# W-Ted/F3D-Gaus

Measured on AMD Instinct MI355X. Metric: rendered views/sec at 256x256 (N Gaussians, K cams), higher is better.
Workload: dtype f32; 1 GPU; C2: 1 image/GPU, 196608 Gaussians (sigma0=0.01), 120-view orbit @256x256, GOF forward raster only; timed region = render + 8-bit RGB frames copied to pinned host memory; compositing arithmetic: fast = error-free float32 pairs for the float64 island + hardware exp/rcp/rsq; every channel within 1e-4 of the oracle (RGB <= 3e-7), EXCEPT that the distortion channel (values 1e-7..1e-5 from cancelling fl; gaussians=196608, views=120, resolution=256, tile_cull=1, views_per_call=120, render_mode=fast, channels=all, parallelism=single GPU

## Files before the change

f3d-gaus_amd/csrc/f3dg_binning.hip:

```cpp
#include "f3dg_common.h"
#include "f3dg_scan.h"

namespace {

typedef unsigned long long u64;
typedef unsigned int u32;

__global__ void __launch_bounds__(F3DG_BLOCK)
scan_reduce_kernel(const u32* __restrict__ in, u64 n, u32* __restrict__ block_sums)
{
    __shared__ u32 wsum[F3DG_BLOCK / 64];
    const u64 base = (u64)blockIdx.x * F3DG_SCAN_CHUNK;
    u32 s = 0;
#pragma unroll
    for (int i = 0; i < F3DG_SCAN_ITEMS; i++) {
        const u64 k = base + (u64)i * F3DG_BLOCK + threadIdx.x;
        if (k < n) s += in[k];
    }
#pragma unroll
    for (int off = 32; off > 0; off >>= 1) s += __shfl_down(s, off, 64);
    if ((threadIdx.x & 63) == 0) wsum[threadIdx.x >> 6] = s;
    __syncthreads();
    if (threadIdx.x == 0) block_sums[blockIdx.x] = wsum[0] + wsum[1] + wsum[2] + wsum[3];
}

__global__ void __launch_bounds__(1024)
scan_blocksums_kernel(u32* __restrict__ block_sums, u32 nblocks, F3dgHeader* __restrict__ hdr)
{
    __shared__ u64 wtot[16];
    const u64 total = scan_array_in_place<16, 1, u64>(block_sums, nblocks, 0u, wtot);
    if (hdr) set_status(hdr, total);
}

__global__ void __launch_bounds__(F3DG_BLOCK)
scan_apply_kernel(const u32* in, u32* out , u64 n, const u32* __restrict__ block_sums,
                  int exclusive)
{
    __shared__ u32 wtot[F3DG_BLOCK / 64];
    const u64 base = (u64)blockIdx.x * F3DG_SCAN_CHUNK + (u64)threadIdx.x * F3DG_SCAN_ITEMS;
    u32 v[F3DG_SCAN_ITEMS];
    u32 s = 0;
    if (base + F3DG_SCAN_ITEMS <= n) {
#pragma unroll
        for (int i = 0; i < F3DG_SCAN_ITEMS / 4; i++) {
            const uint4 w = reinterpret_cast<const uint4*>(in + base)[i];
            v[4 * i] = w.x; v[4 * i + 1] = w.y; v[4 * i + 2] = w.z; v[4 * i + 3] = w.w;
        }
    } else {
#pragma unroll
        for (int i = 0; i < F3DG_SCAN_ITEMS; i++) v[i] = (base + i < n) ? in[base + i] : 0;
    }
#pragma unroll
    for (int i = 0; i < F3DG_SCAN_ITEMS; i++) s += v[i];
    u32 run = block_sums[blockIdx.x] + block_scan_exclusive<F3DG_BLOCK / 64>(s, wtot);
    u32 o[F3DG_SCAN_ITEMS];
#pragma unroll
    for (int i = 0; i < F3DG_SCAN_ITEMS; i++) {
        const u32 before = run;
        run += v[i];
        o[i] = exclusive ? before : run;
    }
    if (base + F3DG_SCAN_ITEMS <= n) {
#pragma unroll
        for (int i = 0; i < F3DG_SCAN_ITEMS / 4; i++)
            reinterpret_cast<uint4*>(out + base)[i] = make_uint4(o[4 * i], o[4 * i + 1], o[4 * i + 2], o[4 * i + 3]);
    } else {
#pragma unroll
        for (int i = 0; i < F3DG_SCAN_ITEMS; i++)
            if (base + i < n) out[base + i] = o[i];
    }
}


struct SegChunk {
    u64 seg_base;
    u64 obase;
    u32 n;
    u32 cps;
    u32 c;
    u32 seg;
};

struct SegTable {
    const u32* vstart;
    const u32* bglob;
    const u32* xprefix;
    u32 xstride;
    u32 V;
};

struct ShiftDigit {
    int shift;
    u32 mask = 255u;
    __device__ __forceinline__ u32 operator()(u32 k) const { return (k >> shift) & mask; }
};
struct CompactDigit {
    u32 kbase;
    __device__ __forceinline__ u32 operator()(u32 k) const { const u32 d = (k - kbase) >> 16; return d < 255u ? d : 255u; }
};

template <typename K, typename DIGIT, bool MINMAX = false>
__device__ __forceinline__ void hist_chunk(const K* __restrict__ keys, const SegChunk& ck, const DIGIT digit, u32* __restrict__ hist,
                                           u32 (*h)[256], u32* __restrict__ minmax = nullptr)
{
    u32 kmin = 0xFFFFFFFFu, kmax = 0u;
#pragma unroll
    for (int w = 0; w < F3DG_BLOCK / 64; w++) h[w][threadIdx.x] = 0;
    __syncthreads();
    u32* hw = h[threadIdx.x >> 6];
    constexpr int VEC = 16 / (int)sizeof(K);
    typedef K __attribute__((ext_vector_type(VEC))) KV;
    const u64 base = (u64)ck.c * F3DG_SORT_CHUNK;
    const u64 g0 = ck.seg_base + base;
    const u64 g1 = ck.seg_base + ((u64)ck.n - base < (u64)F3DG_SORT_CHUNK ? (u64)ck.n : base + F3DG_SORT_CHUNK);
    for (u64 a = (g0 & ~(u64)(VEC - 1)) + (u64)threadIdx.x * VEC; a < g1; a += (u64)F3DG_BLOCK * VEC) {
        const KV w = *reinterpret_cast<const KV*>(keys + a);
#pragma unroll
        for (int q = 0; q < VEC; q++) {
            if (a + q >= g0 && a + q < g1) {
                const u32 key = (u32)w[q];
                atomicAdd(&hw[digit(key)], 1u);
                if (MINMAX && key != 0xFFFFFFFFu) { kmin = key < kmin ? key : kmin; kmax = key > kmax ? key : kmax; }
            }
        }
    }
    __shared__ u32 wmm[2][F3DG_BLOCK / 64];
    if (MINMAX) {
#pragma unroll
        for (int off = 32; off > 0; off >>= 1) {
            const u32 a = __shfl_down(kmin, off, 64), b = __shfl_down(kmax, off, 64);
            kmin = a < kmin ? a : kmin; kmax = b > kmax ? b : kmax;
        }
        if ((threadIdx.x & 63) == 0) { wmm[0][threadIdx.x >> 6] = kmin; wmm[1][threadIdx.x >> 6] = kmax; }
    }
    __syncthreads();
    if (MINMAX && threadIdx.x == 0) {
        u32 a = wmm[0][0], b = wmm[1][0];
#pragma unroll
        for (int w = 1; w < F3DG_BLOCK / 64; w++) { a = wmm[0][w] < a ? wmm[0][w] : a; b = wmm[1][w] > b ? wmm[1][w] : b; }
        minmax[0] = a; minmax[1] = b;
    }
    hist[ck.obase + (u64)threadIdx.x * ck.cps + ck.c] = h[0][threadIdx.x] + h[1][threadIdx.x] + h[2][threadIdx.x] + h[3][threadIdx.x];
}

struct ScatterShared {
    u32 cnt[F3DG_BLOCK / 64][256];
    u32 lbase[256];
    u32 gdelta[256];
    u32 wtot[F3DG_BLOCK / 64];
    u32 sval[F3DG_SORT_CHUNK];
};

template <typename K, bool IOTA, typename DIGIT>
__device__ __forceinline__ void scatter_chunk(const K* __restrict__ keys_in, const u32* __restrict__ vals_in, K* __restrict__ keys_out,
                                              u32* __restrict__ vals_out, const SegChunk& ck, const DIGIT digit,
                                              const u32* __restrict__ offsets , ScatterShared& sh, K* skey)
{
    const u32 n = ck.n;
    const u64 block_base = (u64)ck.c * F3DG_SORT_CHUNK;
    const u32 in_block = (u32)((n - block_base) < (u64)F3DG_SORT_CHUNK ? (n - block_base) : (u64)F3DG_SORT_CHUNK);
    const int lane = threadIdx.x & 63, wave = threadIdx.x >> 6;
#pragma unroll
    for (int w = 0; w < F3DG_BLOCK / 64; w++) sh.cnt[w][threadIdx.x] = 0;
    __syncthreads();

    const u64 wave_base = block_base + (u64)wave * (64 * F3DG_SORT_ITEMS);
    u32 key[F3DG_SORT_ITEMS];
    u32 val[F3DG_SORT_ITEMS];
    u32 rank[F3DG_SORT_ITEMS];
    const u64 lane_lt = ((u64)1 << lane) - 1;
#pragma unroll
    for (int r = 0; r < F3DG_SORT_ITEMS; r++) {
        const u64 i = wave_base + (u64)r * 64 + lane;
        const bool valid = i < n;
        key[r] = valid ? (u32)keys_in[ck.seg_base + i] : 0u;
        val[r] = IOTA ? (u32)i : (valid ? vals_in[ck.seg_base + i] : 0u);
    }
#pragma unroll
    for (int r = 0; r < F3DG_SORT_ITEMS; r++) {
        const u64 i = wave_base + (u64)r * 64 + lane;
        const bool valid = i < n;
        const u32 d = digit(key[r]);
        u64 diff = 0;
#pragma unroll
        for (int b = 0; b < 8; b++) {
            const u32 own = (u32)((int)(d << (31 - b)) >> 31);
            const u64 bal = __ballot(own != 0u);
            diff |= bal ^ (((u64)own << 32) | own);
        }
        const u64 same = __ballot(valid) & ~diff;
        const u32 below = (u32)__popcll(same & lane_lt);
        const u32 prev = sh.cnt[wave][d];
        rank[r] = prev + below;
        __builtin_amdgcn_wave_barrier();
        if (valid && below == 0) sh.cnt[wave][d] = prev + (u32)__popcll(same);
        __builtin_amdgcn_wave_barrier();
    }
    __syncthreads();
    {
        const u32 d = threadIdx.x;
        const u32 c0 = sh.cnt[0][d], c1 = sh.cnt[1][d], c2 = sh.cnt[2][d], c3 = sh.cnt[3][d];
        const u32 tot = c0 + c1 + c2 + c3;
        const u32 excl = block_scan_exclusive<F3DG_BLOCK / 64>(tot, sh.wtot);
        sh.lbase[d] = excl;
        sh.gdelta[d] = offsets[ck.obase + (u64)d * ck.cps + ck.c] - excl;
        sh.cnt[0][d] = excl;
        sh.cnt[1][d] = excl + c0;
        sh.cnt[2][d] = excl + c0 + c1;
        sh.cnt[3][d] = excl + c0 + c1 + c2;
    }
    __syncthreads();
#pragma unroll
    for (int r = 0; r < F3DG_SORT_ITEMS; r++) {
        const u64 i = wave_base + (u64)r * 64 + lane;
        if (i < n) {
            const u32 d = digit(key[r]);
            const u32 slot = sh.cnt[wave][d] + rank[r];
            skey[slot] = (K)key[r];
            sh.sval[slot] = val[r];
        }
    }
    __syncthreads();
    for (u32 slot = threadIdx.x; slot < in_block; slot += F3DG_BLOCK) {
        const K k = skey[slot];
        const u32 d = digit((u32)k);
        const u32 pos = sh.gdelta[d] + slot;
        if (keys_out) keys_out[pos] = k;
        vals_out[pos] = sh.sval[slot];
    }
}

__device__ __forceinline__ SegChunk fixed_chunk(u32 seg_len, u32 cps)
{
    u32 seg, c;
    f3dg_xcd_map(blockIdx.x, gridDim.x / cps, cps, seg, c);
    SegChunk ck;
    ck.seg_base = (u64)seg * seg_len; ck.obase = (u64)seg * 256u * cps; ck.n = seg_len; ck.cps = cps; ck.c = c; ck.seg = seg;
    return ck;
}

__device__ __forceinline__ bool gsort_compact(const u32* __restrict__ minmax, u32 view, u32& kbase)
{
    const u32 kmin = minmax[2 * view], kmax = minmax[2 * view + 1];
    kbase = kmin & 0xFFFF0000u;
    return kmin <= kmax && ((kmax - kbase) >> 24) == 0u;
}

template <int PASS>
__global__ void __launch_bounds__(F3DG_BLOCK)
gsort_hist_kernel(const u32* __restrict__ keys, u32 seg_len, u32 cps, u32* __restrict__ hist, const u32* __restrict__ minmax,
                  u32* __restrict__ chunk_minmax, int standin )
{
    __shared__ u32 h[F3DG_BLOCK / 64][256];
    const SegChunk ck = fixed_chunk(seg_len, cps);
    if constexpr (PASS == 0) {
        hist_chunk<u32, ShiftDigit>(keys, ck, ShiftDigit{0}, hist, h);
    } else if constexpr (PASS == 1) {
        hist_chunk<u32, ShiftDigit, true>(keys, ck, ShiftDigit{8}, hist, h, chunk_minmax + 2 * ((size_t)ck.seg * cps + ck.c));
    } else {
        u32 kbase;
        const bool compact = gsort_compact(minmax, ck.seg, kbase);
        if (!compact) {
            hist_chunk<u32, ShiftDigit>(keys, ck, ShiftDigit{8 * PASS}, hist, h);
        } else if constexpr (PASS == 2) {
            hist_chunk<u32, CompactDigit>(keys, ck, CompactDigit{kbase}, hist, h);
        } else if (standin) {
            const u64 base = (u64)ck.c * F3DG_SORT_CHUNK;
            const u32 in_chunk = (u32)((ck.n - base) < (u64)F3DG_SORT_CHUNK ? (ck.n - base) : (u64)F3DG_SORT_CHUNK);
            hist[ck.obase + (u64)threadIdx.x * ck.cps + ck.c] = threadIdx.x == 0 ? in_chunk : 0u;
        }
    }
}

__global__ void __launch_bounds__(1024)
gsort_scan_kernel(u32 n_per_seg , u32 seg_len, u32* __restrict__ hist, const u32* __restrict__ skip_compact )
{
    __shared__ u32 wtot[16];
    u32 kbase;
    if (skip_compact && gsort_compact(skip_compact, blockIdx.x, kbase)) return;
    scan_array_in_place<16, 4, u32>(hist + (size_t)blockIdx.x * n_per_seg, n_per_seg, blockIdx.x * seg_len, wtot);
}

__global__ void __launch_bounds__(64)
gsort_range_kernel(u32 cps, const u32* __restrict__ chunk_minmax, u32* __restrict__ minmax)
{
    u32 kmin = 0xFFFFFFFFu, kmax = 0u;
    for (u32 c = threadIdx.x; c < cps; c += 64) {
        const u32 a = chunk_minmax[2 * ((size_t)blockIdx.x * cps + c)], b = chunk_minmax[2 * ((size_t)blockIdx.x * cps + c) + 1];
        kmin = a < kmin ? a : kmin; kmax = b > kmax ? b : kmax;
    }
#pragma unroll
    for (int off = 32; off > 0; off >>= 1) {
        const u32 a = __shfl_down(kmin, off, 64), b = __shfl_down(kmax, off, 64);
        kmin = a < kmin ? a : kmin; kmax = b > kmax ? b : kmax;
    }
    if (threadIdx.x == 0) { minmax[2 * blockIdx.x] = kmin; minmax[2 * blockIdx.x + 1] = kmax; }
}

template <int PASS>
__global__ void __launch_bounds__(F3DG_BLOCK)
gsort_scatter_kernel(const u32* __restrict__ keys_in, const u32* __restrict__ vals_in, u32* __restrict__ keys_out,
                     u32* __restrict__ vals_out, u32 seg_len, u32 cps, const u32* __restrict__ offsets, const u32* __restrict__ minmax)
{
    __shared__ ScatterShared sh;
    __shared__ u32 skey[F3DG_SORT_CHUNK];
    const SegChunk ck = fixed_chunk(seg_len, cps);
    if constexpr (PASS == 0) {
        scatter_chunk<u32, true, ShiftDigit>(keys_in, vals_in, keys_out, vals_out, ck, ShiftDigit{0}, offsets, sh, skey);
    } else if constexpr (PASS == 1) {
        scatter_chunk<u32, false, ShiftDigit>(keys_in, vals_in, keys_out, vals_out, ck, ShiftDigit{8}, offsets, sh, skey);
    } else {
        u32 kbase;
        const bool compact = gsort_compact(minmax, ck.seg, kbase);
        if (!compact)
            scatter_chunk<u32, false, ShiftDigit>(keys_in, vals_in, PASS == 3 ? (u32*)nullptr : keys_out, vals_out, ck, ShiftDigit{8 * PASS}, offsets, sh, skey);
        else if constexpr (PASS == 2)
            scatter_chunk<u32, false, CompactDigit>(keys_in, vals_in, (u32*)nullptr, vals_out, ck, CompactDigit{kbase}, offsets, sh, skey);
    }
}


__global__ void __launch_bounds__(1024)
block_sums_scan_kernel(u32 nb, u32* __restrict__ block_sums, u64* __restrict__ view_total)
{
    __shared__ u64 wtot[16];
    const u64 total = scan_array_in_place<16, 1, u64>(block_sums + (size_t)blockIdx.x * nb, nb, 0u, wtot);
    if (threadIdx.x == 0) view_total[blockIdx.x] = total;
}

__global__ void __launch_bounds__(512)
view_segments_kernel(int V, const u64* __restrict__ view_total, F3dgHeader* __restrict__ hdr, u32* __restrict__ vstart,
                     u32* __restrict__ bglob, u32* __restrict__ xprefix, u32 xstride)
{
    __shared__ u64 wtot_v[8];
    __shared__ u32 wtot_c[8];
    const u32 lane = threadIdx.x & 63u, wave = threadIdx.x >> 6;
    u64 total = 0;
    for (u32 v0 = 0; v0 < (u32)V; v0 += 512) {
        const u32 v = v0 + threadIdx.x;
        u64 round;
        const u64 before = block_scan_exclusive<8>(v < (u32)V ? view_total[v] : 0ull, wtot_v, round);
        if (v < (u32)V) vstart[v] = (u32)(total + before);
        total += round;
        __syncthreads();
    }
    const bool dead = set_status(hdr, total);
    if (threadIdx.x == 0) vstart[V] = dead ? 0u : (u32)total;
    if (dead)
        for (u32 v = threadIdx.x; v < (u32)V; v += 512) vstart[v] = 0u;
    __syncthreads();
    auto chunks_of = [&](u32 v) -> u32 {
        const u32 n = vstart[v + 1] - vstart[v];
        return (n + F3DG_SORT_CHUNK - 1) / F3DG_SORT_CHUNK;
    };
    u32 chunks = 0;
    for (u32 v0 = 0; v0 < (u32)V; v0 += 512) {
        const u32 v = v0 + threadIdx.x;
        u32 round;
        const u32 before = block_scan_exclusive<8>(v < (u32)V ? chunks_of(v) : 0u, wtot_c, round);
        if (v < (u32)V) bglob[v] = chunks + before;
        chunks += round;
        __syncthreads();
    }
    if (threadIdx.x == 0) bglob[V] = chunks;
    const u32 nk = ((u32)V > wave) ? ((u32)V - wave + 7u) / 8u : 0u;
    u32 run = 0;
    for (u32 k0 = 0; k0 < nk; k0 += 64) {
        const u32 k = k0 + lane;
        const u32 c = k < nk ? chunks_of(wave + 8u * k) : 0u;
        const u32 x = wave_scan_inclusive(c, lane);
        if (k < nk) xprefix[wave * xstride + k] = run + x - c;
        run += __shfl(x, 63, 64);
    }
    if (lane == 0) xprefix[wave * xstride + nk] = run;
}

__global__ void __launch_bounds__(1024)
tile_scan_kernel(u32 V, const u32* __restrict__ vstart, const u32* __restrict__ bglob, u32* __restrict__ hist)
{
    __shared__ u32 wtot[16];
    const u32 b0 = bglob[blockIdx.x], n = 256u * (bglob[blockIdx.x + 1] - b0);
    if (blockIdx.x == 0 && threadIdx.x == 0) hist[256ull * bglob[V]] = vstart[V];
    scan_array_in_place<16, 16, u32>(hist + 256ull * b0, n, vstart[blockIdx.x], wtot);
}

__global__ void __launch_bounds__(F3DG_BLOCK)
ranges_from_offsets_kernel(u32 V, u32 T, int tile_bits, const u32* __restrict__ bglob, const u32* __restrict__ offsets,
                           const F3dgHeader* __restrict__ hdr, uint2* __restrict__ ranges)
{
    const u32 i = blockIdx.x * F3DG_BLOCK + threadIdx.x;
    if (i >= V * T) return;
    const u32 v = i / T, t = i % T;
    const u32 b0 = bglob[v], cpv = bglob[v + 1] - b0;
    uint2 r = make_uint2(0u, 0u);
    if (cpv != 0u && !hdr->overflow) {
        const u32 d = ((v << tile_bits) | t) & 255u;
        const u32 lo = offsets[256ull * b0 + (u64)d * cpv], hi = offsets[256ull * b0 + (u64)(d + 1u) * cpv];
        if (hi > lo) r = make_uint2(lo, hi);
    }
    ranges[i] = r;
}

__device__ __forceinline__ bool var_chunk(const SegTable& st, u32 f, u32& k, SegChunk& ck)
{
    const u32 x = blockIdx.x & 7u;
    const u32* xp = st.xprefix + x * st.xstride;
    const u32 nk = (st.V > x) ? (st.V - x + 7u) / 8u : 0u;
    while (k < nk && f >= xp[k + 1]) k++;
    if (k >= nk) return false;
    const u32 v = x + 8u * k;
    const u32 s0 = st.vstart[v], b0 = st.bglob[v];
    ck.seg_base = s0; ck.n = st.vstart[v + 1] - s0; ck.cps = st.bglob[v + 1] - b0; ck.obase = 256ull * b0; ck.c = f - xp[k];
    return true;
}

template <typename K>
__global__ void __launch_bounds__(F3DG_BLOCK)
radix2_hist_var_kernel(const K* __restrict__ keys, SegTable st, int shift, u32 mask, u32* __restrict__ hist)
{
    __shared__ u32 h[F3DG_BLOCK / 64][256];
    u32 k = 0;
    SegChunk ck;
    for (u32 f = blockIdx.x >> 3; var_chunk(st, f, k, ck); f += gridDim.x >> 3)
        hist_chunk<K, ShiftDigit>(keys, ck, ShiftDigit{shift, mask}, hist, h);
}

template <typename K>
__global__ void __launch_bounds__(F3DG_BLOCK)
radix2_scatter_var_kernel(const K* __restrict__ keys_in, const u32* __restrict__ vals_in, K* __restrict__ keys_out,
                          u32* __restrict__ vals_out, SegTable st, int shift, u32 mask, const u32* __restrict__ offsets)
{
    __shared__ ScatterShared sh;
    __shared__ K skey[F3DG_SORT_CHUNK];
    u32 k = 0;
    SegChunk ck;
    for (u32 f = blockIdx.x >> 3; var_chunk(st, f, k, ck); f += gridDim.x >> 3) {
        scatter_chunk<K, false, ShiftDigit>(keys_in, vals_in, keys_out, vals_out, ck, ShiftDigit{shift, mask}, offsets, sh, skey);
        __syncthreads();
    }
}

__device__ __forceinline__ u32 rect_instances(u32 x, u32 y)
{
    const u32 rminx = x & F3DG_RECT_COORD, rmaxx = (x >> 16) & F3DG_RECT_COORD, rminy = y & F3DG_RECT_COORD, rmaxy = (y >> 16) & F3DG_RECT_COORD;
    return (rmaxx > rminx && rmaxy > rminy) ? (rmaxx - rminx) * (rmaxy - rminy) : 0u;
}

__global__ void __launch_bounds__(F3DG_BLOCK)
gsort_gather_rects_kernel(int P, u32* __restrict__ gv0, u32* __restrict__ gv1, const u32* __restrict__ minmax,
                          const uint2* __restrict__ rects, u32* __restrict__ block_sums, u32* __restrict__ rx)
{
    constexpr int ITEMS = 4;
    __shared__ u32 wsum[ITEMS][F3DG_BLOCK / 64];
    unsigned view, chunk;
    const unsigned cpv = (unsigned)((P + F3DG_BLOCK * ITEMS - 1) / (F3DG_BLOCK * ITEMS));
    f3dg_xcd_map(blockIdx.x, gridDim.x / cpv, cpv, view, chunk);
    const size_t vb = (size_t)view * P;
    u32 kbase;
    const bool pass2 = gsort_compact(minmax, view, kbase);
    const u32* perm = pass2 ? gv1 : gv0;
    u32* ry = pass2 ? gv0 : gv1;
    const int k0 = (int)(chunk * F3DG_BLOCK * ITEMS + threadIdx.x);
    u32 id[ITEMS];
    uint2 r[ITEMS];
#pragma unroll
    for (int i = 0; i < ITEMS; i++) { const int k = k0 + i * F3DG_BLOCK; id[i] = k < P ? perm[vb + k] : 0u; }
#pragma unroll
    for (int i = 0; i < ITEMS; i++) { const int k = k0 + i * F3DG_BLOCK; r[i] = k < P ? rects[vb + id[i]] : make_uint2(0u, 0u); }
#pragma unroll
    for (int i = 0; i < ITEMS; i++) {
        const int k = k0 + i * F3DG_BLOCK;
        if (k < P) {
            rx[vb + k] = r[i].x;
            ry[vb + k] = r[i].y;
        }
        u32 sum = rect_instances(r[i].x, r[i].y);
#pragma unroll
        for (int off = 32; off > 0; off >>= 1) sum += __shfl_down(sum, off, 64);
        if ((threadIdx.x & 63) == 0) wsum[i][threadIdx.x >> 6] = sum;
    }
    __syncthreads();
    const unsigned nb = (unsigned)((P + F3DG_BLOCK - 1) / F3DG_BLOCK);
    const unsigned blk = chunk * ITEMS + threadIdx.x;
    if (threadIdx.x < ITEMS && blk < nb)
        block_sums[(size_t)view * nb + blk] = wsum[threadIdx.x][0] + wsum[threadIdx.x][1] + wsum[threadIdx.x][2] + wsum[threadIdx.x][3];
}

#define F3DG_DUP_CAP 3072
template <typename G>
__global__ void __launch_bounds__(F3DG_BLOCK)
duplicate_sorted_kernel(int P, int tile_bits, int grid_x, const u32* __restrict__ gv0, const u32* __restrict__ gv1,
                        const u32* __restrict__ minmax, const u32* __restrict__ rx,
                        const u32* __restrict__ block_base , const u32* __restrict__ vstart ,
                        const F3dgHeader* __restrict__ hdr, G* __restrict__ kgrp, u32* __restrict__ vals)
{
    __shared__ G sk[F3DG_DUP_CAP];
    __shared__ u32 sv[F3DG_DUP_CAP];
    __shared__ u32 wtot[F3DG_BLOCK / 64];
    if (hdr->overflow) return;
    const int k = blockIdx.x * F3DG_BLOCK + threadIdx.x;
    const int v = blockIdx.y;
    u32 kbase;
    const bool pass2 = gsort_compact(minmax, (u32)v, kbase);
    const u32* perm = pass2 ? gv1 : gv0;
    const u32* ry = pass2 ? gv0 : gv1;
    const u32 base = (vstart ? vstart[v] : 0u) + block_base[(size_t)v * gridDim.x + blockIdx.x];
    u32 cnt = 0, x = 0, y = 0, g = 0;
    if (k < P) {
        const size_t pos = (size_t)v * P + k;
        x = rx[pos]; y = ry[pos];
        cnt = rect_instances(x, y);
        if (cnt) g = perm[pos];
    }
    u32 n;
    const u32 off0 = block_scan_exclusive<F3DG_BLOCK / 64>(cnt, wtot, n);
    const u32 rminx = x & F3DG_RECT_COORD, rmaxx = (x >> 16) & F3DG_RECT_COORD, rminy = y & F3DG_RECT_COORD, rmaxy = (y >> 16) & F3DG_RECT_COORD;
    const u32 view_base = (u32)v << tile_bits;
    auto halves = [](u32 t, u32 tmin, u32 tmax, u32 word) -> u32 {
        u32 m = 3u;
        if (t == tmin && (word & F3DG_RECT_SKIP_LO)) m &= ~1u;
        if (t + 1u == tmax && (word & F3DG_RECT_SKIP_HI)) m &= ~2u;
        return m;
    };
    for (u32 wb = 0; wb < n; wb += (u32)F3DG_DUP_CAP) {
        const u32 lo = off0 > wb ? off0 : wb;
        const u32 hi = off0 + cnt < wb + (u32)F3DG_DUP_CAP ? off0 + cnt : wb + (u32)F3DG_DUP_CAP;
        if (lo < hi) {
            const u32 w = rmaxx - rminx, j0 = lo - off0;
            u32 ty = rminy + j0 / w, tx = rminx + j0 % w;
            u32 my = halves(ty, rminy, rmaxy, y);
            for (u32 j = lo; j < hi; j++) {
                const u32 mx = halves(tx, rminx, rmaxx, x);
                sk[j - wb] = (G)(view_base | (ty * (u32)grid_x + tx));
                sv[j - wb] = g | ((((my & 1u) ? mx : 0u) | ((my & 2u) ? mx << 2 : 0u)) << F3DG_ID_BITS);
                if (++tx == rmaxx) { tx = rminx; ty++; my = halves(ty, rminy, rmaxy, y); }
            }
        }
        __syncthreads();
        const u32 in_win = n - wb < (u32)F3DG_DUP_CAP ? n - wb : (u32)F3DG_DUP_CAP;
        for (u32 i = threadIdx.x; i < in_win; i += F3DG_BLOCK) {
            kgrp[base + wb + i] = sk[i];
            vals[base + wb + i] = sv[i];
        }
        __syncthreads();
    }
}

__global__ void __launch_bounds__(F3DG_BLOCK)
export_keys_kernel(u32 nseg, int P, int tile_bits, int T, const uint2* __restrict__ ranges, const F3dgHeader* __restrict__ hdr,
                   const u32* __restrict__ point_list, const float* __restrict__ depths, u64* __restrict__ keys_out)
{
    if (hdr->overflow) return;
    for (u32 seg = blockIdx.x; seg < nseg; seg += gridDim.x) {
        const uint2 r = ranges[seg];
        const u32 view = seg / (u32)T, tile = seg % (u32)T;
        const u64 hi = (u64)((view << tile_bits) | tile) << 32;
        for (u32 i = r.x + threadIdx.x; i < r.y; i += F3DG_BLOCK)
            keys_out[i] = hi | (u64)__float_as_uint(depths[(size_t)view * P + (point_list[i] & F3DG_ID_MASK)]);
    }
}

template <typename G>
__global__ void __launch_bounds__(F3DG_BLOCK)
group_bounds_kernel(const G* __restrict__ kgrp, const F3dgHeader* __restrict__ hdr, int tile_bits, int T, u32* __restrict__ ranges)
{
    const u32 L = hdr->overflow ? 0u : hdr->num_rendered;
    const u32 tmask = (1u << tile_bits) - 1u;
    for (u64 base = ((u64)blockIdx.x * F3DG_BLOCK + threadIdx.x) * 8u; base < L; base += (u64)gridDim.x * F3DG_BLOCK * 8u) {
        G v[8];
        if (base + 8 <= L) {
            typedef G __attribute__((ext_vector_type(8))) G8;
            const G8 w = *reinterpret_cast<const G8*>(kgrp + base);
#pragma unroll
            for (int i = 0; i < 8; i++) v[i] = w[i];
        } else {
#pragma unroll
            for (int i = 0; i < 8; i++) v[i] = base + i < L ? kgrp[base + i] : (G)0;
        }
        u32 prev = base > 0 ? (u32)kgrp[base - 1] : 0u;
        const u32 next = base + 8 < L ? (u32)kgrp[base + 8] : 0u;
#pragma unroll
        for (int i = 0; i < 8; i++) {
            const u64 idx = base + i;
            if (idx < L) {
                const u32 cur = (u32)v[i];
                const u32 nxt = i < 7 ? (u32)v[i + 1] : next;
                const u32 seg = (cur >> tile_bits) * (u32)T + (cur & tmask);
                if (idx == 0 || prev != cur) ranges[2u * seg] = (u32)idx;
                if (idx == L - 1 || nxt != cur) ranges[2u * seg + 1u] = (u32)idx + 1u;
                prev = cur;
            }
        }
    }
}

int bits_for(unsigned long long n_values)
{
    int b = 0;
    while (b < 64 && (n_values - 1) >> b) b++;
    return n_values <= 1 ? 0 : b;
}

}

int f3dg_launch_scan_inclusive(hipStream_t s, const unsigned* in, unsigned* out, unsigned long long n,
                               unsigned* tmp, unsigned tmp_elems, int exclusive, F3dgHeader* hdr_total)
{
    if (n == 0) return F3DG_OK;
    const unsigned nblocks = (unsigned)((n + F3DG_SCAN_CHUNK - 1) / F3DG_SCAN_CHUNK);
    if (nblocks > tmp_elems) return F3DG_ERR_WORKSPACE;
    F3DG_KLAUNCH(scan_reduce_kernel, dim3(nblocks), dim3(F3DG_BLOCK), 0, s, in, (u64)n, tmp);
    F3DG_KLAUNCH(scan_blocksums_kernel, dim3(1), dim3(1024), 0, s, tmp, nblocks, hdr_total);
    F3DG_KLAUNCH(scan_apply_kernel, dim3(nblocks), dim3(F3DG_BLOCK), 0, s, in, out, (u64)n, tmp, exclusive);
    F3DG_HIP_CHECK(hipGetLastError());
    return F3DG_OK;
}

int f3dg_tile_bits(int T) { return bits_for((unsigned long long)T); }


int f3dg_sort_passes(int V, int T)
{
    (void)V;
    const int bits = f3dg_tile_bits(T);
    return bits == 0 ? 0 : (bits + 7) / 8;
}

template <typename G>
static int binning_tail(hipStream_t s, int V, int P, int grid_x, int T, int tile_bits, const F3dgLayout& L, char* ws, F3dgHeader* hdr)
{
    int rc = F3DG_OK;
    const size_t VP = (size_t)V * P;
    u32* scan_tmp = reinterpret_cast<u32*>(ws + L.scan_tmp);
    u32* hist = reinterpret_cast<u32*>(ws + L.hist);
    u32* gk[2] = { reinterpret_cast<u32*>(ws + L.gsort), reinterpret_cast<u32*>(ws + L.gsort) + VP };
    u32* gv[2] = { reinterpret_cast<u32*>(ws + L.gsort) + 2 * VP, reinterpret_cast<u32*>(ws + L.gsort) + 3 * VP };
    G* kgrp[2] = { reinterpret_cast<G*>(ws + L.keys[0]), reinterpret_cast<G*>(ws + L.keys[1]) };
    u32* vals[2] = { reinterpret_cast<u32*>(ws + L.vals[0]), reinterpret_cast<u32*>(ws + L.vals[1]) };
    const dim3 pgrid((P + F3DG_BLOCK - 1) / F3DG_BLOCK, V);

    const u32 cps = (u32)((P + F3DG_SORT_CHUNK - 1) / F3DG_SORT_CHUNK);
    const u32 gblocks = (u32)V * cps;
    u32* minmax = reinterpret_cast<u32*>(ws + L.segtab) + L.segtab_minmax;
    u32* chunk_minmax = minmax + 2 * (size_t)V;
    const bool view_scan = cps <= 64;
#define F3DG_GSORT_PASS(PASS, IN, OUT)                                                                                                     \
    F3DG_KLAUNCH((gsort_hist_kernel<PASS>), dim3(gblocks), dim3(F3DG_BLOCK), 0, s, gk[IN], (u32)P, cps, hist, minmax, chunk_minmax, view_scan ? 0 : 1); \
    if (view_scan)                                                                                                                         \
        F3DG_KLAUNCH(gsort_scan_kernel, dim3(V), dim3(1024), 0, s, 256u * cps, (u32)P, hist, PASS == 3 ? minmax : (const u32*)nullptr); \
    else {                                                                                                                                 \
        rc = f3dg_launch_scan_inclusive(s, hist, hist, (unsigned long long)256 * gblocks, scan_tmp, L.scan_tmp_elems, 1, nullptr);        \
        if (rc != F3DG_OK) return rc;                                                                                                      \
    }                                                                                                                                      \
    F3DG_KLAUNCH((gsort_scatter_kernel<PASS>), dim3(gblocks), dim3(F3DG_BLOCK), 0, s, gk[IN], gv[IN], gk[OUT], gv[OUT], (u32)P, cps, hist, minmax)
    F3DG_GSORT_PASS(0, 0, 1);
    F3DG_GSORT_PASS(1, 1, 0);
    F3DG_KLAUNCH(gsort_range_kernel, dim3(V), dim3(64), 0, s, cps, chunk_minmax, minmax);
    F3DG_GSORT_PASS(2, 0, 1);
    F3DG_GSORT_PASS(3, 1, 0);
#undef F3DG_GSORT_PASS
    u32* block_sums = gk[1];
    u32* rx = gk[0];
    u64* view_total = reinterpret_cast<u64*>(chunk_minmax);
    const u32 nb = (u32)((P + F3DG_BLOCK - 1) / F3DG_BLOCK);
    SegTable st;
    u32* segtab = reinterpret_cast<u32*>(ws + L.segtab);
    const u32 xstride = (u32)V / 8u + 2u;
    st.vstart = segtab; st.bglob = segtab + (V + 1); st.xprefix = segtab + 2 * (V + 1); st.xstride = xstride; st.V = (u32)V;

    F3DG_KLAUNCH(gsort_gather_rects_kernel, dim3((unsigned)V * (unsigned)((P + 4 * F3DG_BLOCK - 1) / (4 * F3DG_BLOCK))), dim3(F3DG_BLOCK), 0, s, P, gv[0], gv[1], minmax,
                           reinterpret_cast<const uint2*>(ws + L.rects), block_sums, rx);
    const int passes = f3dg_sort_passes(V, T);
    if (passes > 0) {
        F3DG_KLAUNCH(block_sums_scan_kernel, dim3(V), dim3(1024), 0, s, nb, block_sums, view_total);
        F3DG_KLAUNCH(view_segments_kernel, dim3(1), dim3(512), 0, s, V, view_total, hdr, segtab, segtab + (V + 1), segtab + 2 * (V + 1), xstride);
    } else {
        rc = f3dg_launch_scan_inclusive(s, block_sums, block_sums, (unsigned long long)V * nb, scan_tmp, L.scan_tmp_elems, 1, hdr);
        if (rc != F3DG_OK) return rc;
    }
    int src = passes & 1;
    F3DG_KLAUNCH((duplicate_sorted_kernel<G>), pgrid, dim3(F3DG_BLOCK), 0, s, P, tile_bits, grid_x, gv[0], gv[1], minmax, rx, block_sums,
                       passes > 0 ? segtab : (const u32*)nullptr, hdr, kgrp[src], vals[src]);

    if (passes > 0) {
        const size_t nbmax = (size_t)L.sort_blocks + (size_t)V;
        const u32 per_xcd = (u32)((nbmax + 7) / 8 < 160 ? (nbmax + 7) / 8 : 160);
        const u32 per_xcd_h = (u32)((nbmax + 7) / 8 < 512 ? (nbmax + 7) / 8 : 512);
        const bool tile_view_scan = nbmax <= (size_t)512 * (size_t)V;
        const int split = passes == 2 ? (tile_bits + 1) / 2 : 8;
        for (int p = 0; p < passes; p++) {
            const int shift = split * p;
            const u32 mask = passes == 2 ? (1u << (p == 0 ? split : tile_bits - split)) - 1u : 255u;
            if (!tile_view_scan) F3DG_HIP_CHECK(hipMemsetAsync(hist, 0, sizeof(u32) * 256 * nbmax, s));
            F3DG_KLAUNCH((radix2_hist_var_kernel<G>), dim3(8 * per_xcd_h), dim3(F3DG_BLOCK), 0, s, kgrp[src], st, shift, mask, hist);
            if (tile_view_scan)
                F3DG_KLAUNCH(tile_scan_kernel, dim3(V), dim3(1024), 0, s, (u32)V, st.vstart, st.bglob, hist);
            else {
                rc = f3dg_launch_scan_inclusive(s, hist, hist, (unsigned long long)256 * nbmax, scan_tmp, L.scan_tmp_elems, 1, nullptr);
                if (rc != F3DG_OK) return rc;
            }
            F3DG_KLAUNCH((radix2_scatter_var_kernel<G>), dim3(8 * per_xcd), dim3(F3DG_BLOCK), 0, s, kgrp[src], vals[src],
                               passes == 1 ? (G*)nullptr : kgrp[src ^ 1], vals[src ^ 1], st, shift, mask, hist);
            src ^= 1;
        }
        if (passes == 1) {
            const u32 nseg = (u32)V * (u32)T;
            F3DG_KLAUNCH(ranges_from_offsets_kernel, dim3((nseg + F3DG_BLOCK - 1) / F3DG_BLOCK), dim3(F3DG_BLOCK), 0, s, (u32)V, (u32)T, tile_bits,
                               segtab + (V + 1), hist, hdr, reinterpret_cast<uint2*>(ws + L.ranges));
            F3DG_HIP_CHECK(hipGetLastError());
            return F3DG_OK;
        }
    }
    F3DG_HIP_CHECK(hipMemsetAsync(ws + L.ranges, 0, sizeof(uint2) * (size_t)V * T, s));
    F3DG_KLAUNCH((group_bounds_kernel<G>), dim3(2048), dim3(F3DG_BLOCK), 0, s, kgrp[0], hdr, tile_bits, T, reinterpret_cast<u32*>(ws + L.ranges));
    F3DG_HIP_CHECK(hipGetLastError());
    return F3DG_OK;
}

int f3dg_launch_binning(hipStream_t s, int V, int P, int W, int H, const F3dgLayout& L, char* ws, int export_offsets)
{
    const int grid_x = (W + F3DG_TILE - 1) / F3DG_TILE, grid_y = (H + F3DG_TILE - 1) / F3DG_TILE;
    const int T = grid_x * grid_y;
    const int tile_bits = f3dg_tile_bits(T);
    F3dgHeader* hdr = reinterpret_cast<F3dgHeader*>(ws + L.header);

    int rc = F3DG_OK;
    if (export_offsets) {
        rc = f3dg_launch_scan_inclusive(s, reinterpret_cast<const u32*>(ws + L.tiles), reinterpret_cast<u32*>(ws + L.offsets),
                                        (unsigned long long)V * P, reinterpret_cast<u32*>(ws + L.scan_tmp), L.scan_tmp_elems, 0, nullptr);
        if (rc != F3DG_OK) return rc;
    }
    const bool small = (((unsigned long long)(V > 0 ? V - 1 : 0) << tile_bits) | ((1ull << tile_bits) - 1ull)) <= 0xFFFFull;
    rc = small ? binning_tail<unsigned short>(s, V, P, grid_x, T, tile_bits, L, ws, hdr)
               : binning_tail<u32>(s, V, P, grid_x, T, tile_bits, L, ws, hdr);
    if (rc != F3DG_OK) return rc;
    F3DG_HIP_CHECK(hipGetLastError());
    return F3DG_OK;
}

int f3dg_launch_export_keys(hipStream_t s, int V, int P, int W, int H, const F3dgLayout& L, char* ws)
{
    const int grid_x = (W + F3DG_TILE - 1) / F3DG_TILE, grid_y = (H + F3DG_TILE - 1) / F3DG_TILE;
    const int T = grid_x * grid_y;
    const u32 nseg = (u32)V * (u32)T;
    const u32 rg = nseg < 65535u * 4u ? nseg : 65535u * 4u;
    F3DG_KLAUNCH(export_keys_kernel, dim3(rg), dim3(F3DG_BLOCK), 0, s, nseg, P, f3dg_tile_bits(T), T,
                       reinterpret_cast<const uint2*>(ws + L.ranges), reinterpret_cast<const F3dgHeader*>(ws + L.header),
                       reinterpret_cast<const u32*>(ws + L.vals[0]), reinterpret_cast<const float*>(ws + L.depths),
                       reinterpret_cast<u64*>(ws + L.keys[0]));
    F3DG_HIP_CHECK(hipGetLastError());
    return F3DG_OK;
}
```

Measured before the change: 31080 views/s.

## Narrow radix-sort keys to u16/u8 after first pass and prefetch chunk offsets

The per-view Gaussian depth sort now computes the key range after pass 0. When the range is compact, keys are narrowed to 16-bit and then 8-bit for the later passes, so each scatter and histogram pass reads and writes fewer key bytes. The variable-segment scatter prefetches the next chunk's global offset during the current chunk, and adds a waves-per-EU attribute. The gather kernels load perm and rect values unconditionally with clamped indices so the loads are not predicated. This raises code complexity and depends on the key-range compactness check being correct; the in-place narrow key buffer offsets are subtle.

```diff
diff --git a/f3d-gaus_amd/csrc/f3dg_binning.hip b/f3d-gaus_amd/csrc/f3dg_binning.hip
--- a/f3d-gaus_amd/csrc/f3dg_binning.hip
+++ b/f3d-gaus_amd/csrc/f3dg_binning.hip
@@ -5,6 +5,8 @@
 
 typedef unsigned long long u64;
 typedef unsigned int u32;
+typedef unsigned short u16;
+typedef unsigned char u8;
 
 __global__ void __launch_bounds__(F3DG_BLOCK)
 scan_reduce_kernel(const u32* __restrict__ in, u64 n, u32* __restrict__ block_sums)
@@ -94,10 +96,6 @@
     u32 mask = 255u;
     __device__ __forceinline__ u32 operator()(u32 k) const { return (k >> shift) & mask; }
 };
-struct CompactDigit {
-    u32 kbase;
-    __device__ __forceinline__ u32 operator()(u32 k) const { const u32 d = (k - kbase) >> 16; return d < 255u ? d : 255u; }
-};
 
 template <typename K, typename DIGIT, bool MINMAX = false>
 __device__ __forceinline__ void hist_chunk(const K* __restrict__ keys, const SegChunk& ck, const DIGIT digit, u32* __restrict__ hist,
@@ -151,10 +149,23 @@
     u32 sval[F3DG_SORT_CHUNK];
 };
 
-template <typename K, bool IOTA, typename DIGIT>
-__device__ __forceinline__ void scatter_chunk(const K* __restrict__ keys_in, const u32* __restrict__ vals_in, K* __restrict__ keys_out,
-                                              u32* __restrict__ vals_out, const SegChunk& ck, const DIGIT digit,
-                                              const u32* __restrict__ offsets , ScatterShared& sh, K* skey)
+struct KeepKey {
+    __device__ __forceinline__ u32 operator()(u32 k) const { return k; }
+};
+struct Narrow16 {
+    u32 kbase;
+    __device__ __forceinline__ u32 operator()(u32 k) const { return k == 0xFFFFFFFFu ? 0xFFFFu : (k - kbase) >> 8; }
+};
+struct Narrow8 {
+    __device__ __forceinline__ u32 operator()(u32 k) const { return k >> 8; }
+};
+
+__device__ __forceinline__ u64 chunk_offset_entry(const SegChunk& ck) { return ck.obase + (u64)threadIdx.x * ck.cps + ck.c; }
+
+template <typename K, typename KO, bool IOTA, typename DIGIT, typename NARROW>
+__device__ __forceinline__ void scatter_chunk(const K* __restrict__ keys_in, const u32* __restrict__ vals_in, KO* __restrict__ keys_out,
+                                              u32* __restrict__ vals_out, const SegChunk& ck, const DIGIT digit, const NARROW narrow,
+                                              const u32* __restrict__ offsets , u32& goff, const SegChunk* next, ScatterShared& sh, K* skey)
 {
     const u32 n = ck.n;
     const u64 block_base = (u64)ck.c * F3DG_SORT_CHUNK;
@@ -203,7 +214,7 @@
         const u32 tot = c0 + c1 + c2 + c3;
         const u32 excl = block_scan_exclusive<F3DG_BLOCK / 64>(tot, sh.wtot);
         sh.lbase[d] = excl;
-        sh.gdelta[d] = offsets[ck.obase + (u64)d * ck.cps + ck.c] - excl;
+        sh.gdelta[d] = goff - excl;
         sh.cnt[0][d] = excl;
         sh.cnt[1][d] = excl + c0;
         sh.cnt[2][d] = excl + c0 + c1;
@@ -221,11 +232,12 @@
         }
     }
     __syncthreads();
+    if (next) goff = offsets[chunk_offset_entry(*next)];
     for (u32 slot = threadIdx.x; slot < in_block; slot += F3DG_BLOCK) {
         const K k = skey[slot];
         const u32 d = digit((u32)k);
         const u32 pos = sh.gdelta[d] + slot;
-        if (keys_out) keys_out[pos] = k;
+        if (keys_out) keys_out[pos] = (KO)narrow((u32)k);
         vals_out[pos] = sh.sval[slot];
     }
 }
@@ -239,6 +251,18 @@
     return ck;
 }
 
+template <typename K>
+__device__ __forceinline__ SegChunk narrow_chunk(SegChunk ck)
+{
+    ck.seg_base *= 4u / (u32)sizeof(K);
+    return ck;
+}
+template <typename K>
+__device__ __forceinline__ K* gsort_keys(const u32* keys, const SegChunk& ck)
+{
+    return reinterpret_cast<K*>(const_cast<u32*>(keys)) + ck.seg_base * (4u / (u32)sizeof(K) - 1u);
+}
+
 __device__ __forceinline__ bool gsort_compact(const u32* __restrict__ minmax, u32 view, u32& kbase)
 {
     const u32 kmin = minmax[2 * view], kmax = minmax[2 * view + 1];
@@ -254,16 +278,16 @@
     __shared__ u32 h[F3DG_BLOCK / 64][256];
     const SegChunk ck = fixed_chunk(seg_len, cps);
     if constexpr (PASS == 0) {
-        hist_chunk<u32, ShiftDigit>(keys, ck, ShiftDigit{0}, hist, h);
-    } else if constexpr (PASS == 1) {
-        hist_chunk<u32, ShiftDigit, true>(keys, ck, ShiftDigit{8}, hist, h, chunk_minmax + 2 * ((size_t)ck.seg * cps + ck.c));
+        hist_chunk<u32, ShiftDigit, true>(keys, ck, ShiftDigit{0}, hist, h, chunk_minmax + 2 * ((size_t)ck.seg * cps + ck.c));
     } else {
         u32 kbase;
         const bool compact = gsort_compact(minmax, ck.seg, kbase);
         if (!compact) {
             hist_chunk<u32, ShiftDigit>(keys, ck, ShiftDigit{8 * PASS}, hist, h);
+        } else if constexpr (PASS == 1) {
+            hist_chunk<u16, ShiftDigit>(reinterpret_cast<const u16*>(keys), narrow_chunk<u16>(ck), ShiftDigit{0}, hist, h);
         } else if constexpr (PASS == 2) {
-            hist_chunk<u32, CompactDigit>(keys, ck, CompactDigit{kbase}, hist, h);
+            hist_chunk<u8, ShiftDigit>(reinterpret_cast<const u8*>(keys), narrow_chunk<u8>(ck), ShiftDigit{0}, hist, h);
         } else if (standin) {
             const u64 base = (u64)ck.c * F3DG_SORT_CHUNK;
             const u32 in_chunk = (u32)((ck.n - base) < (u64)F3DG_SORT_CHUNK ? (ck.n - base) : (u64)F3DG_SORT_CHUNK);
@@ -305,17 +329,21 @@
     __shared__ ScatterShared sh;
     __shared__ u32 skey[F3DG_SORT_CHUNK];
     const SegChunk ck = fixed_chunk(seg_len, cps);
-    if constexpr (PASS == 0) {
-        scatter_chunk<u32, true, ShiftDigit>(keys_in, vals_in, keys_out, vals_out, ck, ShiftDigit{0}, offsets, sh, skey);
+    u32 goff = offsets[chunk_offset_entry(ck)];
+    u32 kbase;
+    const bool compact = gsort_compact(minmax, ck.seg, kbase);
+    if (!compact) {
+        scatter_chunk<u32, u32, PASS == 0, ShiftDigit, KeepKey>(keys_in, vals_in, PASS == 3 ? (u32*)nullptr : keys_out, vals_out, ck, ShiftDigit{8 * PASS},
+                                                                KeepKey{}, offsets, goff, nullptr, sh, skey);
+    } else if constexpr (PASS == 0) {
+        scatter_chunk<u32, u16, true, ShiftDigit, Narrow16>(keys_in, vals_in, gsort_keys<u16>(keys_out, ck), vals_out, ck, ShiftDigit{0}, Narrow16{kbase},
+                                                            offsets, goff, nullptr, sh, skey);
     } else if constexpr (PASS == 1) {
-        scatter_chunk<u32, false, ShiftDigit>(keys_in, vals_in, keys_out, vals_out, ck, ShiftDigit{8}, offsets, sh, skey);
-    } else {
-        u32 kbase;
-        const bool compact = gsort_compact(minmax, ck.seg, kbase);
-        if (!compact)
-            scatter_chunk<u32, false, ShiftDigit>(keys_in, vals_in, PASS == 3 ? (u32*)nullptr : keys_out, vals_out, ck, ShiftDigit{8 * PASS}, offsets, sh, skey);
-        else if constexpr (PASS == 2)
-            scatter_chunk<u32, false, CompactDigit>(keys_in, vals_in, (u32*)nullptr, vals_out, ck, CompactDigit{kbase}, offsets, sh, skey);
+        scatter_chunk<u16, u8, false, ShiftDigit, Narrow8>(gsort_keys<u16>(keys_in, ck), vals_in, gsort_keys<u8>(keys_out, ck), vals_out, ck, ShiftDigit{0},
+                                                           Narrow8{}, offsets, goff, nullptr, sh, reinterpret_cast<u16*>(skey));
+    } else if constexpr (PASS == 2) {
+        scatter_chunk<u8, u8, false, ShiftDigit, KeepKey>(gsort_keys<u8>(keys_in, ck), vals_in, (u8*)nullptr, vals_out, ck, ShiftDigit{0}, KeepKey{},
+                                                          offsets, goff, nullptr, sh, reinterpret_cast<u8*>(skey));
     }
 }
 
@@ -426,17 +454,24 @@
 }
 
 template <typename K>
-__global__ void __launch_bounds__(F3DG_BLOCK)
+__global__ void __launch_bounds__(F3DG_BLOCK) __attribute__((amdgpu_waves_per_eu(4, 4)))
 radix2_scatter_var_kernel(const K* __restrict__ keys_in, const u32* __restrict__ vals_in, K* __restrict__ keys_out,
                           u32* __restrict__ vals_out, SegTable st, int shift, u32 mask, const u32* __restrict__ offsets)
 {
     __shared__ ScatterShared sh;
     __shared__ K skey[F3DG_SORT_CHUNK];
-    u32 k = 0;
-    SegChunk ck;
-    for (u32 f = blockIdx.x >> 3; var_chunk(st, f, k, ck); f += gridDim.x >> 3) {
-        scatter_chunk<K, false, ShiftDigit>(keys_in, vals_in, keys_out, vals_out, ck, ShiftDigit{shift, mask}, offsets, sh, skey);
+    const u32 stride = gridDim.x >> 3;
+    u32 k = 0, f = blockIdx.x >> 3;
+    SegChunk ck, next;
+    bool live = var_chunk(st, f, k, ck);
+    u32 goff = live ? offsets[chunk_offset_entry(ck)] : 0u;
+    while (live) {
+        u32 kn = k;
+        const bool more = var_chunk(st, f + stride, kn, next);
+        scatter_chunk<K, K, false, ShiftDigit, KeepKey>(keys_in, vals_in, keys_out, vals_out, ck, ShiftDigit{shift, mask}, KeepKey{}, offsets, goff,
+                                                        more ? &next : (const SegChunk*)nullptr, sh, skey);
         __syncthreads();
+        ck = next; k = kn; f += stride; live = more;
     }
 }
 
@@ -464,12 +499,14 @@
     u32 id[ITEMS];
     uint2 r[ITEMS];
 #pragma unroll
-    for (int i = 0; i < ITEMS; i++) { const int k = k0 + i * F3DG_BLOCK; id[i] = k < P ? perm[vb + k] : 0u; }
-#pragma unroll
-    for (int i = 0; i < ITEMS; i++) { const int k = k0 + i * F3DG_BLOCK; r[i] = k < P ? rects[vb + id[i]] : make_uint2(0u, 0u); }
+    for (int i = 0; i < ITEMS; i++) { const int k = k0 + i * F3DG_BLOCK; id[i] = perm[vb + (k < P ? k : P - 1)]; }
+#pragma unroll
+    for (int i = 0; i < ITEMS; i++) r[i] = rects[vb + id[i]];
 #pragma unroll
     for (int i = 0; i < ITEMS; i++) {
         const int k = k0 + i * F3DG_BLOCK;
+        const u32 live = k < P ? 0xFFFFFFFFu : 0u;
+        r[i].x &= live; r[i].y &= live;
         if (k < P) {
             rx[vb + k] = r[i].x;
             ry[vb + k] = r[i].y;
@@ -508,9 +545,8 @@
     u32 cnt = 0, x = 0, y = 0, g = 0;
     if (k < P) {
         const size_t pos = (size_t)v * P + k;
-        x = rx[pos]; y = ry[pos];
+        x = rx[pos]; y = ry[pos]; g = perm[pos];
         cnt = rect_instances(x, y);
-        if (cnt) g = perm[pos];
     }
     u32 n;
     const u32 off0 = block_scan_exclusive<F3DG_BLOCK / 64>(cnt, wtot, n);
@@ -652,10 +688,11 @@
         rc = f3dg_launch_scan_inclusive(s, hist, hist, (unsigned long long)256 * gblocks, scan_tmp, L.scan_tmp_elems, 1, nullptr);        \
         if (rc != F3DG_OK) return rc;                                                                                                      \
     }                                                                                                                                      \
+    if (PASS == 0)                \
+        F3DG_KLAUNCH(gsort_range_kernel, dim3(V), dim3(64), 0, s, cps, chunk_minmax, minmax);                                            \
     F3DG_KLAUNCH((gsort_scatter_kernel<PASS>), dim3(gblocks), dim3(F3DG_BLOCK), 0, s, gk[IN], gv[IN], gk[OUT], gv[OUT], (u32)P, cps, hist, minmax)
     F3DG_GSORT_PASS(0, 0, 1);
     F3DG_GSORT_PASS(1, 1, 0);
-    F3DG_KLAUNCH(gsort_range_kernel, dim3(V), dim3(64), 0, s, cps, chunk_minmax, minmax);
     F3DG_GSORT_PASS(2, 0, 1);
     F3DG_GSORT_PASS(3, 1, 0);
 #undef F3DG_GSORT_PASS
```

Result: faster. 31960 views/s, median of 6 (+2.8%).
